# zhoubin-me/agent0

Hardware: AMD Instinct MI355X
Metric: env-frames/sec (learner FPS: transitions collected and saved to replay per second with the learner running, pre-frameskip) (higher is better)
Workload: dtype f32

## Files before the change

agent0_amd/csrc/encoder_fused.hip:

```cpp
#include "a0_internal.h"
#include "net_tables.h"
#include "operands.h"
#include "store_policy.h"
#include "update_tail.h"

#include <cstdlib>
#include <type_traits>

typedef float a0_acc4 __attribute__((ext_vector_type(4)));

struct a0_fused_args {
    const uint8_t* frames; const int* slot; long long sample_stride; int chan_off;
    const float *wt1, *wt2, *wt3;
    const float *wx2, *wx3;
    const float *b1, *b2, *b3;
    float *act1, *act2, *act3;
    int B;
    int C, H, W, H1, W1, H2, W2, H3, W3;
    int off_act1, off_act2, off_end;
    int rp1, rp2;
};

A0_HD void a0_fused_set_wt(a0_fused_args& P, const float* wt, int C) {
    const a0_wt_layout T{C};
// ... 357 lines not shown
    const float* bias; uint16_t* planes; float* glb; int N;
    A0_D void emit_n4(int m, int n0, const a0_acc4& acc, const float*) const {
        const a0_f4 bv = *(const a0_f4*)(bias + n0);
        float v[4] = {acc[0] + bv.x, acc[1] + bv.y, acc[2] + bv.z, acc[3] + bv.w};
#pragma unroll
        for (int r = 0; r < 4; ++r) v[r] = (v[r] < 0.f) ? 0.f : v[r];
        if (glb) *(a0_f4*)(glb + (unsigned)(m * N + n0)) = a0_f4{v[0], v[1], v[2], v[3]};
        uint2 hi, mid, lo;
        a0_split4(v, hi, mid, lo);
        const int oh = m / OWC;
        uint16_t* d = planes + oh * RP + (m - oh * OWC) * P + n0;
        *(uint2*)d = hi; *(uint2*)(d + term) = mid; *(uint2*)(d + 2 * term) = lo;
    }
};
struct EpiFwdT {
    static constexpr bool PER_ELEM = false;
    static constexpr bool ROW4 = false;
    static constexpr bool TR = true;
    const float* bias; float* glb; int N;
    A0_D void emit_n4(int m, int n0, const a0_acc4& acc, const float*) const {
        const a0_f4 bv = *(const a0_f4*)(bias + n0);
        float v[4] = {acc[0] + bv.x, acc[1] + bv.y, acc[2] + bv.z, acc[3] + bv.w};
#pragma unroll
        for (int r = 0; r < 4; ++r) v[r] = (v[r] < 0.f) ? 0.f : v[r];
        *(a0_f4*)(glb + (unsigned)(m * N + n0)) = a0_f4{v[0], v[1], v[2], v[3]};
    }
};

template <int ORD, int N, int WN, int MBT, int R, int LR, class AFX, class EPI, class Between>
A0_D void a0_conv_stage_x9k(const AFX& af, int M, a0_wring9<N, WN, R, A0_FUSED_WAVES / WN>& ring, const EPI& epi, float* xch0, float* xch1, Between&& between) {
    constexpr int WK = A0_FUSED_WAVES / WN, HB0 = (MBT + 1) / 2, HB1 = MBT / 2;
    static_assert(WK == 2 && N == 16 * WN && HB1 >= 1 && EPI::TR && LR >= 1 && LR <= 16, "tile shape");
    const int tid = threadIdx.x, lane = tid & 63;
    const int wave = __builtin_amdgcn_readfirstlane(tid >> 6);
    const int wn = wave % WN, wk = wave / WN;
    const int q = lane >> 4, r16 = lane & 15;
    const int MB = (M + 15) >> 4, NSTW = ring.nst;
    int rows[MBT];
#pragma unroll
    for (int i = 0; i < MBT; ++i) {
        const int m = i * 16 + r16;
        rows[i] = af.row(m < M ? m : 0) + 8 * q;
    }
    a0_acc4 acc[MBT];
#pragma unroll
    for (int i = 0; i < MBT; ++i) acc[i] = a0_acc4{0.f, 0.f, 0.f, 0.f};
    uint4 a[2][HB0][3];
    auto fetch = [&](int slot, int h, int off) {
#pragma unroll
        for (int i = 0; i < HB0; ++i)
            if (h * HB0 + i < MBT) {
#pragma unroll
                for (int t = 0; t < 3; ++t) a[slot][i][t] = *(const uint4*)(af.planes + rows[h * HB0 + i] + off + t * AFX::term);
            }
    };
    fetch(0, 0, af.step_off(wk));
    __builtin_amdgcn_s_waitcnt(0x0F70);
#pragma unroll 1
    for (int tb = 0; tb < NSTW; tb += R) {
#pragma unroll
        for (int u = 0; u < R; ++u) {
            const int st = wk + WK * (tb + u);
            const int off = af.step_off(st), offn = af.step_off(tb + u + 1 < NSTW ? st + WK : st);
#pragma unroll
            for (int h = 0; h < 2; ++h) {
                if (h == 0) fetch(1, 1, off);
                else fetch(0, 0, offn);
                __builtin_amdgcn_sched_barrier(0);
#pragma unroll
                for (int ta = 0; ta < 3; ++ta)
#pragma unroll
                    for (int tw = 0; tw < 3; ++tw)
#pragma unroll
                        for (int i = 0; i < HB0; ++i) {
                            if (ta + tw > ORD || h * HB0 + i >= MBT) continue;
                            const a0_u32x4 av = {a[h][i][ta].x, a[h][i][ta].y, a[h][i][ta].z, a[h][i][ta].w};
                            const a0_u32x4 bv = {ring.v[u][0][tw].x, ring.v[u][0][tw].y, ring.v[u][0][tw].z, ring.v[u][0][tw].w};
                            acc[h * HB0 + i] = __builtin_amdgcn_mfma_f32_16x16x32_bf16(__builtin_bit_cast(a0_bf16x8, bv), __builtin_bit_cast(a0_bf16x8, av), acc[h * HB0 + i], 0, 0, 0);
                        }
                __builtin_amdgcn_sched_barrier(0);
            }
            ring.fill(u);
            __builtin_amdgcn_sched_barrier(0);
        }
    }
    between();
    a0_acc4* x0 = (a0_acc4*)xch0;
    a0_acc4* x1 = (a0_acc4*)xch1;
    constexpr int P1 = (HB1 - 1) * 64 + 4 * LR;
    const int last = q * LR + r16;
    const int n0 = wn * 16 + 4 * q;
    float pe[EPI::PER_ELEM ? HB0 : 1][4];
    auto send = [&](auto mine) {
        constexpr int H = decltype(mine)::value;
        if constexpr (EPI::PER_ELEM) {
#pragma unroll
            for (int i = 0; i < (H == 0 ? HB0 : HB1); ++i) {
                const int m = (H * HB0 + i) * 16 + r16;
                const a0_f4 v = epi.pre_elem4(m < M ? m : M - 1, n0);
                pe[i][0] = v.x; pe[i][1] = v.y; pe[i][2] = v.z; pe[i][3] = v.w;
            }
        }
        if constexpr (H == 1) {
#pragma unroll
            for (int i = 0; i < HB0; ++i) x0[(wn * HB0 + i) * 64 + lane] = acc[i];
        } else {
#pragma unroll
            for (int i = 0; i < HB1; ++i) {
                if (i < HB1 - 1) x1[wn * P1 + i * 64 + lane] = acc[HB0 + i];
                else if (r16 < LR) x1[wn * P1 + (HB1 - 1) * 64 + last] = acc[HB0 + i];
            }
        }
    };
    auto recv = [&](auto mine) {
        constexpr int H = decltype(mine)::value;
#pragma unroll
        for (int i = 0; i < (H == 0 ? HB0 : HB1); ++i) {
            const int mb = H * HB0 + i;
            const int m = mb * 16 + r16;
            if constexpr (H == 0) acc[mb] += x0[(wn * HB0 + i) * 64 + lane];
            else {
                if (i < HB1 - 1) acc[mb] += x1[wn * P1 + i * 64 + lane];
                else if (r16 < LR) acc[mb] += x1[wn * P1 + (HB1 - 1) * 64 + last];
            }
            if (mb < MB && m < M) epi.emit_n4(m, n0, acc[mb], EPI::PER_ELEM ? pe[EPI::PER_ELEM ? i : 0] : nullptr);
        }
    };
    if (wk == 0) send(std::integral_constant<int, 0>{});
    else send(std::integral_constant<int, 1>{});
    __syncthreads();
    if (wk == 0) recv(std::integral_constant<int, 0>{});
    else recv(std::integral_constant<int, 1>{});
    __syncthreads();
}
constexpr int A0_P1X = 40, A0_P2X = 80;
constexpr int A0_RP1X = 20 * A0_P1X + 8;
constexpr int A0_RP2X = 9 * A0_P2X + 96;

constexpr int A0_R1 = 4, A0_R2 = 4, A0_R3 = 6;

template <int MBW1, int MBW2, int MBW3, int WC, bool X9, bool LOOP = false, int ORD = 4>
__global__ __launch_bounds__(A0_FUSED_THREADS) void a0_encoder_fused_kernel(a0_fused_args P);

constexpr int A0_X9_BIAS_OFF = 2 * 4 * 84 * 84 + 3 * 20 * A0_RP1X * 2;
constexpr int A0_RK2 = 2, A0_RK3 = 3;
constexpr int A0_X9_XCH0 = 3 * 9 * A0_RP2X * 2;
constexpr int A0_X9_XCH1 = A0_X9_BIAS_OFF + 160 * 4;
static_assert(A0_X9_XCH0 + 4 * 3 * 1024 <= 2 * 4 * 84 * 84, "conv2 exchange region 0 fits into the image");
constexpr int A0_X9_LDS_BYTES = A0_X9_XCH1 + 4 * (2 * 64 + 4) * 16;
static_assert(A0_X9_LDS_BYTES <= 160 * 1024, "LDS");
static_assert(A0_FUSED_WAVES == 8, "N-stationary stages: four waves along N, two along K");
typedef a0_wring9<64, 4, A0_RK2, 2> a0_ring2_t;
typedef a0_wring9<64, 4, A0_RK3, 2> a0_ring3_t;
template <int ORD, bool LOOP>
A0_D void a0_x9_conv23(const a0_fused_args& P, int b, unsigned char* smem, float* bias_lds, a0_wring1<A0_R1>& ring1, a0_ring2_t& ring2, a0_ring3_t& ring3) {
    const int obs_bytes = P.C * P.H * P.W;
    const int M2 = P.H2 * P.W2, M3 = P.H3 * P.W3;
    uint16_t* a1p = (uint16_t*)(smem + 2 * obs_bytes);
    constexpr int term1 = 20 * A0_RP1X, term2 = 9 * A0_RP2X;
    uint16_t* a2p = (uint16_t*)smem;
    typedef EpiFwdX<9, A0_P2X, A0_RP2X, term2> E2X;
    const AF2X<term1> f2{a1p, A0_RP1X, P.W2, A0_P1X};
    const E2X e2{bias_lds + 32, a2p, P.act2 ? P.act2 + (long long)b * M2 * 64 : nullptr, 64};
    const AF3X<term2> f3{a2p, A0_RP2X, P.W3, A0_P2X};
    const EpiFwdT e3{bias_lds + 96, P.act3 + (long long)b * M3 * 64, 64};
    a0_conv_stage_x9k<ORD, 64, 4, 6, A0_RK2, 1>(f2, M2, ring2, e2, (float*)(smem + A0_X9_XCH0), (float*)(smem + A0_X9_XCH1), [&] { ring3.prologue(); });
    a0_conv_stage_x9k<ORD, 64, 4, 4, A0_RK3, 16>(f3, M3, ring3, e3, (float*)a1p, (float*)a1p + 4 * 2 * 256, [&] { if (LOOP) ring1.prologue(); });
}

A0_D void a0_bytes16_to_img(uint16_t* img, int idx16, const uint4& v) {
    const uint32_t w[4] = {v.x, v.y, v.z, v.w};
    uint32_t o[8];
#pragma unroll
    for (int k = 0; k < 4; ++k) {
        const uint32_t f0 = __float_as_uint((float)(w[k] & 0xffu)), f1 = __float_as_uint((float)((w[k] >> 8) & 0xffu));
        const uint32_t f2 = __float_as_uint((float)((w[k] >> 16) & 0xffu)), f3 = __float_as_uint((float)(w[k] >> 24));
        o[2 * k] = __builtin_amdgcn_perm(f1, f0, 0x07060302u);
        o[2 * k + 1] = __builtin_amdgcn_perm(f3, f2, 0x07060302u);
    }
    ((uint4*)img)[2 * idx16] = uint4{o[0], o[1], o[2], o[3]};
    ((uint4*)img)[2 * idx16 + 1] = uint4{o[4], o[5], o[6], o[7]};
}

template <int ORD, bool LOOP>
A0_D void a0_encoder_fused_x9_body(const a0_fused_args& P, int bid, int nblk) {
    extern __shared__ __attribute__((aligned(16))) unsigned char smem[];
    uint16_t* img = (uint16_t*)smem;
    const int obs_bytes = P.C * P.H * P.W;
    const int M1 = P.H1 * P.W1;
    uint16_t* a1p = (uint16_t*)(smem + 2 * obs_bytes);
    constexpr int term1 = 20 * A0_RP1X;
    typedef EpiFwdX<20, A0_P1X, A0_RP1X, term1> E1X;
    a0_wring1<A0_R1> ring1;
    a0_ring2_t ring2;
    a0_ring3_t ring3;
    ring1.init(P.wt1, P.C);
    ring2.init(P.wx2, 512);
    ring3.init(P.wx3, 576);
    ring1.prologue();
    constexpr int MBW1X = (25 + A0_WMG1 - 1) / A0_WMG1;
    a0_pre<32, 2, MBW1X, E1X> pre1;
    float* bias_lds = (float*)(smem + A0_X9_BIAS_OFF);
    if (threadIdx.x < 160) bias_lds[threadIdx.x] = threadIdx.x < 32 ? P.b1[threadIdx.x] : threadIdx.x < 96 ? P.b2[threadIdx.x - 32] : P.b3[threadIdx.x - 96];
    for (int b = bid; b < P.B; b += nblk) {
        const long long s = P.slot ? (long long)P.slot[b] : (long long)b;
        const uint4* src = (const uint4*)(P.frames + s * P.sample_stride + P.chan_off);
        constexpr int TRIPS = 4;
        const int n16 = obs_bytes >> 4;
        for (int i0 = threadIdx.x; i0 < n16; i0 += TRIPS * A0_FUSED_THREADS) {
            uint4 v[TRIPS];
#pragma unroll
            for (int j = 0; j < TRIPS; ++j) {
                const int i = i0 + j * A0_FUSED_THREADS;
                v[j] = src[i < n16 ? i : n16 - 1];
            }
#pragma unroll
            for (int j = 0; j < TRIPS; ++j) {
                const int i = i0 + j * A0_FUSED_THREADS;
                a0_bytes16_to_img(img, i < n16 ? i : n16 - 1, v[j]);
            }
        }
        __syncthreads();
        const E1X e1{bias_lds, a1p, P.act1 ? P.act1 + (long long)b * M1 * 32 : nullptr, 32};
        const int wmg1 = __builtin_amdgcn_readfirstlane(threadIdx.x >> 6) / 2;
        if (MBW1X > 1 && wmg1 + (MBW1X - 1) * A0_WMG1 >= ((M1 + 15) >> 4))
            a0_conv1_stage<(MBW1X > 1 ? MBW1X - 1 : 1), A0_R1, 84>(img, P.H * P.W, P.W, P.W1, M1, ring1, e1, pre1, [&] { ring2.prologue(); });
        else
            a0_conv1_stage<MBW1X, A0_R1, 84>(img, P.H * P.W, P.W, P.W1, M1, ring1, e1, pre1, [&] { ring2.prologue(); });
        a0_x9_conv23<ORD, LOOP>(P, b, smem, bias_lds, ring1, ring2, ring3);
        if constexpr (!LOOP) break;
    }
}

#include "actor_tail.h"
typedef a0_st_nt a0_step_row_store;
struct a0_step_enc_args { const float *wt, *b1, *b2, *b3; float* act3; };
template <int ORD>
__global__ __launch_bounds__(A0_FUSED_THREADS) void a0_actor_dist_step_enc_kernel(a0_dtenv_args Q, a0_step_enc_args N) {
    __shared__ int s_chase_cell;
    extern __shared__ __attribute__((aligned(16))) unsigned char smem[];
    unsigned long long v_wt = (unsigned long long)N.wt, v_b1 = (unsigned long long)N.b1, v_b2 = (unsigned long long)N.b2, v_b3 = (unsigned long long)N.b3,
                       v_a3 = (unsigned long long)N.act3, v_obs = (unsigned long long)Q.obs_out;
    A0_TO_VGPR(v_wt); A0_TO_VGPR(v_b1); A0_TO_VGPR(v_b2); A0_TO_VGPR(v_b3); A0_TO_VGPR(v_a3); A0_TO_VGPR(v_obs);
    int v_E = Q.E;
    A0_TO_VGPR(v_E);
    a0_actor_dist_tail_env_body(Q, (float*)smem, &s_chase_cell);
    __syncthreads();
    auto uni = [](unsigned long long v) {
        return ((unsigned long long)(unsigned)__builtin_amdgcn_readfirstlane((int)(v >> 32)) << 32) | (unsigned long long)(unsigned)__builtin_amdgcn_readfirstlane((int)(v & 0xffffffffull));
    };
    const float* wt = (const float*)uni(v_wt);
    a0_fused_args P;
    P.frames = (const uint8_t*)uni(v_obs); P.slot = nullptr; P.sample_stride = 4 * 84 * 84; P.chan_off = 0;
    a0_fused_set_wt(P, wt, 4);
    P.b1 = (const float*)uni(v_b1); P.b2 = (const float*)uni(v_b2); P.b3 = (const float*)uni(v_b3);
    P.act1 = nullptr; P.act2 = nullptr; P.act3 = (float*)uni(v_a3); P.B = __builtin_amdgcn_readfirstlane(v_E);
    P.C = 4; P.H = 84; P.W = 84; P.H1 = 20; P.W1 = 20; P.H2 = 9; P.W2 = 9; P.H3 = 7; P.W3 = 7;
    P.off_act1 = 0; P.off_act2 = 0; P.off_end = 0; P.rp1 = 0; P.rp2 = 0;
    a0_encoder_fused_x9_body<ORD, false>(P, (int)blockIdx.x, (int)gridDim.x);
}

template <int MBW, class EPI, class Mid, class Between>
A0_D void a0_conv1_stage_split(const uint16_t* img, a0_wring1<A0_R1>& ring, const EPI& epi, bool first_before_mid, Mid&& mid, Between&& between) {
    static_assert(A0_R1 == 4 && EPI::TR, "ring of four steps, transposed accumulators");
    constexpr int HW = 84 * 84, W = 84, W1 = 20, M = 400, MB = 25;
    const int tid = threadIdx.x, lane = tid & 63;
    const int wave = __builtin_amdgcn_readfirstlane(tid >> 6);
    const int wn = wave % 2, wmg = wave / 2;
    const int q = lane >> 4, r16 = lane & 15;
    int rows[MBW];
#pragma unroll
    for (int i = 0; i < MBW; ++i) {
        int m = (wmg + i * A0_WMG1) * 16 + r16;
        m = m < M ? m : 0;
        const int oh = m / W1, ow = m - oh * W1;
        rows[i] = (4 * oh + q) * W + 4 * ow;
    }
    a0_acc4 acc[MBW];
#pragma unroll
    for (int i = 0; i < MBW; ++i) acc[i] = a0_acc4{0.f, 0.f, 0.f, 0.f};
    uint2 a[2][MBW][2];
    auto fetch = [&](int slot, int off) {
#pragma unroll
        for (int i = 0; i < MBW; ++i) {
            a[slot][i][0] = *(const uint2*)(img + rows[i] + off);
            a[slot][i][1] = *(const uint2*)(img + rows[i] + off + 4);
        }
    };
    auto off_of = [&](int st) { return (st >> 1) * HW + (st & 1) * 4 * W; };
    auto step = [&](auto UC, int off_next) {
        constexpr int u = decltype(UC)::value;
        fetch((u + 1) & 1, off_next);
        __builtin_amdgcn_sched_barrier(0);
#pragma unroll
        for (int s3 = 0; s3 < 3; ++s3)
#pragma unroll
            for (int i = 0; i < MBW; ++i) {
                const a0_u32x4 av = {a[u & 1][i][0].x, a[u & 1][i][0].y, a[u & 1][i][1].x, a[u & 1][i][1].y};
                const a0_u32x4 bv = {ring.v[u][s3].x, ring.v[u][s3].y, ring.v[u][s3].z, ring.v[u][s3].w};
                acc[i] = __builtin_amdgcn_mfma_f32_16x16x32_bf16(__builtin_bit_cast(a0_bf16x8, bv), __builtin_bit_cast(a0_bf16x8, av), acc[i], 0, 0, 0);
            }
        __builtin_amdgcn_sched_barrier(0);
        ring.fill(u);
        __builtin_amdgcn_sched_barrier(0);
    };
    typedef std::integral_constant<int, 0> U0; typedef std::integral_constant<int, 1> U1; typedef std::integral_constant<int, 2> U2; typedef std::integral_constant<int, 3> U3;
    auto steps05 = [&] {
        fetch(0, off_of(0));
        __builtin_amdgcn_s_waitcnt(0x0F70);
        step(U0{}, off_of(1)); step(U1{}, off_of(2)); step(U2{}, off_of(3)); step(U3{}, off_of(4));
        step(U0{}, off_of(5)); step(U1{}, off_of(5));
    };
    if (first_before_mid) steps05();
    mid();
    if (!first_before_mid) steps05();
    fetch(0, off_of(6));
    __builtin_amdgcn_s_waitcnt(0x0F70);
    step(U2{}, off_of(7)); step(U3{}, off_of(7));
    between();
#pragma unroll
    for (int i = 0; i < MBW; ++i) {
        const int mb = wmg + i * A0_WMG1;
        if (mb < MB) {
            const int m = mb * 16 + r16;
            if (m < M) epi.emit_n4(m, wn * 16 + 4 * q, acc[i], nullptr);
        }
    }
    __syncthreads();
}

struct TailScalar {
    typedef a0_qenv_args Args;
    static A0_D void run(const a0_qenv_args& Q, uint32_t e, uint32_t g, long long steps, unsigned long long off_a, unsigned long long off_u, float eps, long long slot, const a0_u4& x,
                         bool chase, int lane, float* w2s , float* raw, int* s_chase_cell_p) {
        const int NQ = Q.A + (Q.dueling ? 1 : 0);
// ... 46 lines not shown
    if (tid < 160) bias_lds[tid] = tid < 32 ? P.b1[tid] : tid < 96 ? P.b2[tid - 32] : P.b3[tid - 96];
    unsigned long long v_wx2 = (unsigned long long)P.wx2, v_wx3 = (unsigned long long)P.wx3;
    A0_TO_VGPR(v_wx2); A0_TO_VGPR(v_wx3);
    uint32_t g = Q.g; long long steps = Q.steps, start = Q.start; unsigned long long off_a = Q.off_a, off_u = Q.off_u; float eps = Q.eps;
    if (Q.ctrl) {
        g += (uint32_t)Q.ctrl[A0_CTRL_ENV_STEP]; steps += Q.ctrl[A0_CTRL_ACTOR_STEPS]; start += Q.ctrl[A0_CTRL_REPLAY_SLOT];
        off_a += (unsigned long long)Q.ctrl[A0_CTRL_RNG_ACTION]; off_u += (unsigned long long)Q.ctrl[A0_CTRL_RNG_UNIFORM];
    }
    eps = a0_env_eps(eps, Q.eps_ptr, e);
    const long long slot = (start + e) % Q.cap;
    uint32_t e_v = e;
    asm volatile("" : "+v"(e_v));
    const a0_u4 x = a0_philox4x32_10(e_v, g, 0u, 0x454E56u, (uint32_t)Q.env_seed, (uint32_t)(Q.env_seed >> 32) ^ Q.rank);
    const bool term = __builtin_amdgcn_readfirstlane((int)((x.y % 500u) == 0u)) != 0;
    const bool chase = Q.task == A0_ENV_TASK_CHASE;
    const bool early = !(chase && term);
    const int j = tid - 64;
    auto has_group = [&] { int jj = j; asm volatile("" : "+v"(jj)); return wave != 0 && jj < G16; };
    const uint32_t pbase = (uint32_t)Q.env_seed ^ a0_env_mix32(e * 0x9E3779B1u + g);
    uint4* out16 = (uint4*)(Q.obs_out + (size_t)e * 4 * HW) + j;
    uint4* row16 = (uint4*)(Q.frames + slot * (8LL * HW)) + j;
    A0_TO_VGPR(out16); A0_TO_VGPR(row16);
    float* act3_v = N.act3;
    A0_TO_VGPR(act3_v);
    auto new_group = [&](uint32_t by, uint32_t bx) {
        uint32_t w[4];
#pragma unroll
        for (int k = 0; k < 4; ++k) {
            const uint32_t p = 16u * (uint32_t)j + 4u * (uint32_t)k;
            w[k] = (uint32_t)a0_env_pixel(pbase, by, bx, p, chase) | ((uint32_t)a0_env_pixel(pbase, by, bx, p + 1, chase) << 8) |
                   ((uint32_t)a0_env_pixel(pbase, by, bx, p + 2, chase) << 16) | ((uint32_t)a0_env_pixel(pbase, by, bx, p + 3, chase) << 24);
        }
        return uint4{w[0], w[1], w[2], w[3]};
    };
    auto put = [&](int c, const uint4 v) {
        out16[c * G16] = v; a0_store16<a0_step_row_store>(row16 + (4 + c) * G16, v);
        a0_bytes16_to_img(img, c * G16 + j, v);
    };
    __shared__ int s_staged;
    if (tid == 0) s_staged = 0;
    __syncthreads();
    uint4 keep[9];
    if (wave == 0) {
        TAIL::run(Q, e, g, steps, off_a, off_u, eps, slot, x, chase, lane, (float*)a1p, raw, &s_chase_cell);
    } else {
        if (has_group()) {
            const uint4* in16 = (const uint4*)(Q.obs_in + (size_t)e * 4 * HW) + j;
            A0_TO_VGPR(in16);
            const uint4 i0 = in16[0], i1 = in16[G16], i2 = in16[2 * G16], i3 = in16[3 * G16];
            if (Q.obs0 == Q.obs_in) { keep[0] = i0; keep[1] = i1; keep[2] = i2; keep[3] = i3; }
            else {
                const uint4* o016 = (const uint4*)(Q.obs0 + (size_t)e * 4 * HW) + j;
                A0_TO_VGPR(o016);
                keep[0] = o016[0]; keep[1] = o016[G16]; keep[2] = o016[2 * G16]; keep[3] = o016[3 * G16];
            }
            if (!chase) {
                const uint4 nw = new_group((3u * g + 11u * e) % 77u, (5u * g + 7u * e) % 77u);
                if (term) { keep[4] = nw; keep[5] = nw; keep[6] = nw; } else { keep[4] = i1; keep[5] = i2; keep[6] = i3; }
                keep[7] = nw;
                for (int c = 0; c < 4; ++c) a0_bytes16_to_img(img, c * G16 + j, keep[4 + c]);
            } else if (!term) {
                keep[4] = i1; keep[5] = i2; keep[6] = i3;
                for (int c = 0; c < 3; ++c) a0_bytes16_to_img(img, c * G16 + j, keep[4 + c]);
            }
        }
        asm volatile("s_waitcnt lgkmcnt(0)" ::: "memory");
        if (lane == 0) atomicAdd(&s_staged, 1);
        while (__builtin_amdgcn_readfirstlane(*(volatile int*)&s_staged) < A0_FUSED_WAVES - 1) __builtin_amdgcn_s_sleep(1);
    }
    auto early_stores = [&] {
        if (has_group()) {
#pragma unroll
            for (int c = 0; c < 4; ++c) a0_store16<a0_step_row_store>(row16 + c * G16, keep[c]);
            const int nc = !chase ? 4 : (!term ? 3 : 0);
#pragma unroll
            for (int c = 0; c < 4; ++c)
                if (c < nc) { out16[c * G16] = keep[4 + c]; a0_store16<a0_step_row_store>(row16 + (4 + c) * G16, keep[4 + c]); }
        }
    };
    auto mid = [&] {
        if (wave != 0) early_stores();
        __syncthreads();
        if (chase) {
            if (has_group()) {
                uint32_t by, bx;
                a0_chase_pos(s_chase_cell, by, bx);
                const uint4 nw = new_group(by, bx);
                if (term) { put(0, nw); put(1, nw); put(2, nw); }
                put(3, nw);
            }
            __syncthreads();
        }
    };
    auto uni = [](unsigned long long v) {
        return ((unsigned long long)(unsigned)__builtin_amdgcn_readfirstlane((int)(v >> 32)) << 32) | (unsigned long long)(unsigned)__builtin_amdgcn_readfirstlane((int)(v & 0xffffffffull));
    };
    ring2.init((const float*)uni(v_wx2), 512);
    ring3.init((const float*)uni(v_wx3), 576);
    typedef EpiFwdX<20, A0_P1X, A0_RP1X, 20 * A0_RP1X> E1X;
    const E1X e1{bias_lds, a1p, nullptr, 32};
    constexpr int MBW1X = (25 + A0_WMG1 - 1) / A0_WMG1;
    const bool before = early && wave != 0;
    if (MBW1X > 1 && wave / 2 + (MBW1X - 1) * A0_WMG1 >= 25)
        a0_conv1_stage_split<(MBW1X > 1 ? MBW1X - 1 : 1)>(img, ring1, e1, before, mid, [&] { ring2.prologue(); });
    else
        a0_conv1_stage_split<MBW1X>(img, ring1, e1, before, mid, [&] { ring2.prologue(); });
    P.act3 = (float*)uni((unsigned long long)act3_v);
    a0_x9_conv23<ORD, false>(P, (int)e, smem, bias_lds, ring1, ring2, ring3);
}

template <int ORD>
__global__ __launch_bounds__(A0_FUSED_THREADS) void a0_actor_step_enc2_kernel(a0_qenv_args Q, a0_step_enc_args N) { a0_actor_step_enc2_body<ORD, TailScalar>(Q, N); }

static bool a0_fused_layout(int C, int H, int W, a0_fused_args& P, size_t& lds_bytes);
int a0_actor_dist_step_enc_launch(const a0_dtenv_args& Q, size_t tail_lds, const float* wt, const a0_encoder_weights* w, float* act3, hipStream_t st) {
    a0_fused_args P;
    size_t lds = 0;
    if (!wt || !w || !w->b1 || !w->b2 || !w->b3 || !act3 || !a0_fused_layout(4, 84, 84, P, lds)) return a0_fail(A0_EINVAL, "a0_actor_dist_tail_env_step_enc: bad encoder argument");
    if (P.H1 != 20 || P.W1 != 20 || P.H2 != 9 || P.W2 != 9 || P.H3 != 7 || P.W3 != 7) return a0_fail(A0_EINVAL, "a0_actor_dist_tail_env_step_enc: geometry");
    const a0_step_enc_args N{wt, w->b1, w->b2, w->b3, act3};
    lds = A0_X9_LDS_BYTES > tail_lds ? (size_t)A0_X9_LDS_BYTES : tail_lds;
    if (lds > 160 * 1024 - 64) return a0_fail(A0_EINVAL, "a0_actor_dist_tail_env_step_enc: head too wide for LDS");
    const int six = a0_x9_products_now() == 6;
    auto kern = six ? a0_actor_dist_step_enc_kernel<2> : a0_actor_dist_step_enc_kernel<4>;
    static size_t configured[2] = {0, 0};
    if (lds > configured[six]) {
        if (hipFuncSetAttribute((const void*)kern, hipFuncAttributeMaxDynamicSharedMemorySize, (int)lds) != hipSuccess)
            return a0_fail(A0_EINVAL, "a0_actor_dist_tail_env_step_enc: LDS");
        configured[six] = lds;
    }
    A0_LAUNCH_PROBED(A0_TAG_ACTOR_STEP_ENC, 2.0 * (400.0 * 32 * 256 + 81.0 * 64 * 512 + 49.0 * 64 * 576) * Q.E, kern, dim3(Q.E), dim3(A0_FUSED_THREADS), lds, st, Q, N);
    return a0_fail_hip((int)hipGetLastError(), "a0_actor_dist_tail_env_step_enc");
}
int a0_actor_step_enc_launch(const a0_qenv_args& Q, const float* wt, const a0_encoder_weights* w, float* act3, hipStream_t st) {
    a0_fused_args P;
    size_t lds = 0;
    if (!wt || !w || !w->b1 || !w->b2 || !w->b3 || !act3 || !a0_fused_layout(4, 84, 84, P, lds)) return a0_fail(A0_EINVAL, "a0_actor_qhead_env_step_enc: bad encoder argument");
    if (P.H1 != 20 || P.W1 != 20 || P.H2 != 9 || P.W2 != 9 || P.H3 != 7 || P.W3 != 7) return a0_fail(A0_EINVAL, "a0_actor_qhead_env_step_enc: geometry");
    const a0_step_enc_args N{wt, w->b1, w->b2, w->b3, act3};
    const size_t tail_lds = (size_t)(Q.A + (Q.dueling ? 1 : 0)) * 512 * sizeof(float);
    lds = A0_X9_LDS_BYTES > tail_lds ? (size_t)A0_X9_LDS_BYTES : tail_lds;
    const int six = a0_x9_products_now() == 6;
    auto kern = six ? a0_actor_step_enc2_kernel<2> : a0_actor_step_enc2_kernel<4>;
    static size_t configured[2] = {0, 0};
    if (lds > configured[six]) {
        if (hipFuncSetAttribute((const void*)kern, hipFuncAttributeMaxDynamicSharedMemorySize, (int)lds) != hipSuccess)
            return a0_fail(A0_EINVAL, "a0_actor_qhead_env_step_enc: LDS");
        configured[six] = lds;
    }
    A0_LAUNCH_PROBED(A0_TAG_ACTOR_STEP_ENC, 2.0 * (400.0 * 32 * 256 + 81.0 * 64 * 512 + 49.0 * 64 * 576) * Q.E, kern, dim3(Q.E), dim3(A0_FUSED_THREADS), lds, st, Q, N);
    return a0_fail_hip((int)hipGetLastError(), "a0_actor_qhead_env_step_enc");
}

struct a0_fused_multi_args { a0_fused_args p[3]; int first[4]; };
template <int ORD>
__global__ __launch_bounds__(A0_FUSED_THREADS) void a0_encoder_fused_multi_kernel(a0_fused_multi_args M) {
    const int bid = (int)blockIdx.x;
    const int k = bid >= M.first[2] ? 2 : (bid >= M.first[1] ? 1 : 0);
    a0_encoder_fused_x9_body<ORD, true>(M.p[k], bid - M.first[k], M.first[k + 1] - M.first[k]);
}

template <int MBW1, int MBW2, int MBW3, int WC, bool X9, bool LOOP, int ORD>
__global__ __launch_bounds__(A0_FUSED_THREADS) void a0_encoder_fused_kernel(a0_fused_args P) {
    if constexpr (X9) {
        static_assert(MBW1 == 7 && MBW2 == 3 && MBW3 == 2 && WC == 84, "the split-operand body is written for the 4 x 84 x 84 geometry");
        a0_encoder_fused_x9_body<ORD, LOOP>(P, (int)blockIdx.x, (int)gridDim.x);
        return;
    }
    extern __shared__ __attribute__((aligned(16))) unsigned char smem[];
    uint16_t* img = (uint16_t*)smem;
    float* fl = (float*)smem;
    float* act1 = fl + P.off_act1;
    float* act2 = fl + P.off_act2;
    const int obs_bytes = P.C * P.H * P.W;
    const int M1 = P.H1 * P.W1, M2 = P.H2 * P.W2, M3 = P.H3 * P.W3;
    a0_wring1<A0_R1> ring1;
    a0_wring<64, 4, A0_R2> ring2;
    a0_wring<64, 4, A0_R3> ring3;
    ring1.init(P.wt1, P.C);
    ring2.init(P.wt2, 512);
    ring3.init(P.wt3, 576);
    ring1.prologue();
    constexpr int OW1 = WC == 84 ? 20 : 0, OW2 = WC == 84 ? 9 : 0;
    a0_pre<32, 2, MBW1, EpiFwd<OW1>> pre1;
    a0_pre<64, 4, MBW2, EpiFwd<OW2>> pre2;
    a0_pre<64, 4, MBW3, EpiFwd<0>> pre3;
    pre1.load(EpiFwd<OW1>{P.b1, nullptr, 0, 0, 1, nullptr, 32}, M1);
    pre2.load(EpiFwd<OW2>{P.b2, nullptr, 0, 0, 1, nullptr, 64}, M2);
    pre3.load(EpiFwd<0>{P.b3, nullptr, 0, 0, 1, nullptr, 64}, M3);
    for (int b = blockIdx.x; b < P.B; b += gridDim.x) {
        const long long s = P.slot ? (long long)P.slot[b] : (long long)b;
        const uint4* src = (const uint4*)(P.frames + s * P.sample_stride + P.chan_off);
        constexpr int TRIPS = 4;
        const int n16 = obs_bytes >> 4;
        for (int i0 = threadIdx.x; i0 < n16; i0 += TRIPS * A0_FUSED_THREADS) {
            uint4 v[TRIPS];
#pragma unroll
            for (int j = 0; j < TRIPS; ++j) {
                const int i = i0 + j * A0_FUSED_THREADS;
                v[j] = src[i < n16 ? i : n16 - 1];
            }
#pragma unroll
            for (int j = 0; j < TRIPS; ++j) {
                const int i = i0 + j * A0_FUSED_THREADS;
                a0_bytes16_to_img(img, i < n16 ? i : n16 - 1, v[j]);
            }
        }
        __syncthreads();
        const EpiFwd<OW1> e1{P.b1, act1, A0_P1, P.rp1, P.W1, P.act1 ? P.act1 + (long long)b * M1 * 32 : nullptr, 32};
        const int wmg1 = __builtin_amdgcn_readfirstlane(threadIdx.x >> 6) / 2;
        if (MBW1 > 1 && wmg1 + (MBW1 - 1) * 4 >= ((M1 + 15) >> 4))
            a0_conv1_stage<(MBW1 > 1 ? MBW1 - 1 : 1), A0_R1, WC>(img, P.H * P.W, P.W, P.W1, M1, ring1, e1, pre1, [&] { ring2.prologue(); });
        else
            a0_conv1_stage<MBW1, A0_R1, WC>(img, P.H * P.W, P.W, P.W1, M1, ring1, e1, pre1, [&] { ring2.prologue(); });
        AF2 f2{act1, P.rp1, P.W2};
        const EpiFwd<OW2> e2{P.b2, act2, A0_P2, P.rp2, P.W2, P.act2 ? P.act2 + (long long)b * M2 * 64 : nullptr, 64};
        a0_conv_stage<64, 4, MBW2, 3, A0_R2>(f2, M2, 512, ring2, e2, pre2, [&] { ring3.prologue(); });
        AF3 f3{act2, P.rp2, P.W3};
        const EpiFwd<0> e3{P.b3, nullptr, 0, 0, 1, P.act3 + (long long)b * M3 * 64, 64};
        a0_conv_stage<64, 4, MBW3, 3, A0_R3>(f3, M3, 576, ring3, e3, pre3, [&] { ring1.prologue(); });
    }
}

struct a0_dgrad_args {
    const float *d3, *act1, *act2;
    float *d2, *d1;
    const float *wd3, *wd2;
    int B;
};
constexpr int A0_RPDA = 11 * A0_P2X + 96, A0_RPDB = 11 * A0_P2X + 48;
constexpr int A0_DTERMA = 11 * A0_RPDA, A0_DTERMB = 11 * A0_RPDB;
struct AFD3X {
    static constexpr int term = A0_DTERMA;
    const uint16_t* planes;
    A0_D int row(int m) const { const int oh = m / 9, ow = m - oh * 9; return oh * A0_RPDA + ow * A0_P2X; }
    A0_D int step_off(int st) const { const int tap = st >> 1; return (tap / 3) * A0_RPDA + (tap % 3) * A0_P2X + 32 * (st & 1); }
};
struct AFD2X {
    static constexpr int term = A0_DTERMB;
    const uint16_t* planes;
    A0_D int row(int m) const { const int oh = m / 10, ow = m - oh * 10; return oh * A0_RPDB + ow * A0_P2X; }
    A0_D int step_off(int st) const { const int cell = st >> 1; return (cell >> 1) * A0_RPDB + (cell & 1) * A0_P2X + 32 * (st & 1); }
};
struct EpiBwd3X {
    static constexpr bool PER_ELEM = true;
    static constexpr bool ROW4 = false;
    static constexpr bool TR = true;
    const float* mask; float* dst; uint16_t* planes;
    A0_D a0_f4 pre_elem4(int m, int n0) const { return *(const a0_f4*)(mask + (unsigned)(m * 64 + n0)); }
    A0_D void emit_n4(int m, int n0, const a0_acc4& acc, const float* pre) const {
        float v[4];
#pragma unroll
        for (int r = 0; r < 4; ++r) v[r] = pre[r] > 0.f ? acc[r] : 0.f;
        *(a0_f4*)(dst + (unsigned)(m * 64 + n0)) = a0_f4{v[0], v[1], v[2], v[3]};
        uint2 hi, mid, lo;
        a0_split4(v, hi, mid, lo);
        const int oh = m / 9, ow = m - oh * 9;
        uint16_t* d = planes + (oh + 1) * A0_RPDB + (ow + 1) * A0_P2X + n0;
        *(uint2*)d = hi; *(uint2*)(d + A0_DTERMB) = mid; *(uint2*)(d + 2 * A0_DTERMB) = lo;
    }
};
static_assert((A0_RPDB % 4) == 0 && (A0_DTERMB % 4) == 0 && (A0_P2X % 4) == 0, "8-byte aligned plane writes");
struct EpiBwdPair {
    static constexpr bool PER_ELEM = true;
    static constexpr bool ROW4 = false;
    static constexpr bool TR = true;
    const float* mask; float* dst; int p0;
    A0_D unsigned gi(int m, int n0) const {
        const int p = p0 + (n0 >> 5), oh = m / 10, ow = m - oh * 10;
        return (unsigned)(((oh * 2 + (p >> 1)) * 20 + ow * 2 + (p & 1)) * 32 + (n0 & 31));
    }
    A0_D a0_f4 pre_elem4(int m, int n0) const { return *(const a0_f4*)(mask + gi(m, n0)); }
    A0_D void emit_n4(int m, int n0, const a0_acc4& acc, const float* pre) const {
        *(a0_f4*)(dst + gi(m, n0)) = a0_f4{pre[0] > 0.f ? acc[0] : 0.f, pre[1] > 0.f ? acc[1] : 0.f, pre[2] > 0.f ? acc[2] : 0.f, pre[3] > 0.f ? acc[3] : 0.f};
    }
};
template <int ORD>
__global__ __launch_bounds__(A0_FUSED_THREADS) void a0_encoder_dgrad_fused_x9_kernel(a0_dgrad_args P) {
    extern __shared__ __attribute__((aligned(16))) unsigned char smem[];
    uint16_t* plA = (uint16_t*)smem;
    uint16_t* plB = plA + 3 * A0_DTERMA;
    for (int i = threadIdx.x; i < 3 * (A0_DTERMA + A0_DTERMB) / 2; i += A0_FUSED_THREADS) ((uint32_t*)smem)[i] = 0u;
    float* const xch0 = (float*)(smem + 3 * (A0_DTERMA + A0_DTERMB) * 2);
    float* const xch1 = xch0 + 4 * 4 * 256;
    const int lane = threadIdx.x & 63, wave = __builtin_amdgcn_readfirstlane(threadIdx.x >> 6), wn = wave & 3, wk = wave >> 2;
    a0_wring9<64, 4, 3, 2> ring3;
    a0_wring9<64, 4, 2, 2> ringq[2];
    ring3.init(P.wd3, 576);
    ring3.prologue();
    const uint4* const wq = (const uint4*)P.wd2 + (((wn & 1) * 16 + (lane & 15)) * 4 + (lane >> 4)) * 3 + (wn >> 1) * 3072 + wk * 384;
    __syncthreads();
    for (int b = blockIdx.x; b < P.B; b += gridDim.x) {
        const a0_f4* src = (const a0_f4*)(P.d3 + (long long)b * 49 * 64);
        for (int i = threadIdx.x; i < 49 * 16; i += A0_FUSED_THREADS) {
            const a0_f4 v = src[i];
            const int pos = i >> 4, c4 = (i & 15) * 4, h = pos / 7, w = pos - h * 7;
            const float x[4] = {v.x, v.y, v.z, v.w};
            uint2 hi, mid, lo;
            a0_split4(x, hi, mid, lo);
            uint16_t* d = plA + (h + 2) * A0_RPDA + (w + 2) * A0_P2X + c4;
            *(uint2*)(d) = hi; *(uint2*)(d + A0_DTERMA) = mid; *(uint2*)(d + 2 * A0_DTERMA) = lo;
        }
        __syncthreads();
        const AFD3X f3{plA};
        const AFD2X f2{plB};
        const EpiBwd3X e3{P.act2 + (long long)b * 81 * 64, P.d2 + (long long)b * 81 * 64, plB};
        const EpiBwdPair e2a{P.act1 + (long long)b * 400 * 32, P.d1 + (long long)b * 400 * 32, 0};
        const EpiBwdPair e2b{P.act1 + (long long)b * 400 * 32, P.d1 + (long long)b * 400 * 32, 2};
        a0_conv_stage_x9k<ORD, 64, 4, 6, 3, 1>(f3, 81, ring3, e3, xch0, xch1, [&] { ringq[0].init_at(wq, 4, 768); ringq[0].prologue(); });
        a0_conv_stage_x9k<ORD, 64, 4, 7, 2, 4>(f2, 100, ringq[0], e2a, xch0, xch1, [&] { ringq[1].init_at(wq + 2 * 3072, 4, 768); ringq[1].prologue(); });
        a0_conv_stage_x9k<ORD, 64, 4, 7, 2, 4>(f2, 100, ringq[1], e2b, xch0, xch1, [&] { ring3.prologue(); });
    }
}

__global__ void a0_conv_wt_kernel(const float* __restrict__ w1, const float* __restrict__ w2, const float* __restrict__ w3, float* __restrict__ wt, int K1,
                                  float* __restrict__ wt2, const int* __restrict__ state, int* __restrict__ commit) {
    const bool mirror = wt2 != nullptr && state[4] != 0;
    if (commit != nullptr && blockIdx.x == 0 && threadIdx.x == 0) { commit[1] = commit[5]; commit[0] = 0; }
    const a0_wt_layout T{K1 / 64};
    const int i = blockIdx.x * blockDim.x + threadIdx.x;
    if (i >= T.total()) return;
    uint32_t out = 0;
    if (i >= T.conv2() && i < T.conv2x()) {
        const bool c3 = i >= T.conv3();
        const int e = i - (c3 ? T.conv3() : T.conv2());
        const int j = e & 3, q = (e >> 2) & 3, n = (e >> 4) & 63, k = 16 * (e >> 10) + 4 * j + q;
        out = __float_as_uint(c3 ? w3[n * 576 + k] : w2[n * 512 + k]);
    } else {
        enum { CONV1, CONV2, CONV3, DGRAD3, DGRAD2 } seg;
        int e, N = 64, phase = 0;
        if (i < T.conv2()) { seg = CONV1; e = i; N = 32; }
        else if (i < T.conv3x()) { seg = CONV2; e = i - T.conv2x(); }
        else if (i < T.dgrad3x()) { seg = CONV3; e = i - T.conv3x(); }
        else if (i < T.dgrad2x()) { seg = DGRAD3; e = i - T.dgrad3x(); }
        else { seg = DGRAD2; e = i - T.dgrad2x(); phase = e / T.n_dgrad2x_phase; e -= phase * T.n_dgrad2x_phase; N = 32; }
        const int pair = e & 3, f = e >> 2, s = f % 3, q = (f / 3) & 3, n = (f / 12) % N, t = f / (12 * N);
        for (int h = 0; h < 2; ++h) {
            const int k = 32 * t + 8 * q + 2 * pair + h, cell = k >> 6, co = k & 63;
            float w;
            if (seg == CONV1) w = w1[n * K1 + k] / 255.0f;
            else if (seg == CONV2) w = w2[n * 512 + k];
            else if (seg == CONV3) w = w3[n * 576 + k];
            else if (seg == DGRAD3) {
                const int kh = 2 - cell / 3, kw = 2 - cell % 3;
                w = w3[co * 576 + (kh * 3 + kw) * 64 + n];
            } else {
                const int kh = (phase >> 1) + 2 * (1 - (cell >> 1)), kw = (phase & 1) + 2 * (1 - (cell & 1));
                w = w2[co * 512 + (kh * 4 + kw) * 32 + n];
            }
            out |= a0_bf16_term(w, s) << (16 * h);
        }
    }
    *(uint32_t*)(wt + i) = out;
    if (mirror) *(uint32_t*)(wt2 + i) = out;
}

extern "C" long long a0_net_conv_wt_floats(int C) { return a0_wt_layout{C}.total(); }

extern "C" int a0_net_conv_wt_refresh(const a0_encoder_weights* w, int C, float* wt, void* stream) {
    if (!w || !w->w1 || !w->w2 || !w->w3 || !wt || C < 1) return a0_fail(A0_EINVAL, "a0_net_conv_wt_refresh: bad argument");
    const long long n = a0_net_conv_wt_floats(C);
    hipLaunchKernelGGL(a0_conv_wt_kernel, dim3((unsigned)((n + 255) / 256)), dim3(256), 0, (hipStream_t)stream, w->w1, w->w2, w->w3, wt, C * 64, (float*)nullptr,
                       (const int*)nullptr, (int*)nullptr);
    return a0_fail_hip((int)hipGetLastError(), "a0_net_conv_wt_refresh");
}

extern "C" int a0_net_conv_wt_refresh_sync(const a0_encoder_weights* w, int C, float* wt, float* wt_target, const int* state, void* stream) {
    if (!w || !w->w1 || !w->w2 || !w->w3 || !wt || !wt_target || !state || C < 1) return a0_fail(A0_EINVAL, "a0_net_conv_wt_refresh_sync: bad argument");
    const long long n = a0_net_conv_wt_floats(C);
    hipLaunchKernelGGL(a0_conv_wt_kernel, dim3((unsigned)((n + 255) / 256)), dim3(256), 0, (hipStream_t)stream, w->w1, w->w2, w->w3, wt, C * 64, wt_target, state, (int*)nullptr);
    return a0_fail_hip((int)hipGetLastError(), "a0_net_conv_wt_refresh_sync");
}

int a0_conv_wt_refresh_commit(const a0_encoder_weights* w, int C, float* wt, float* wt_target, int* state, hipStream_t st) {
    if (!w || !w->w1 || !w->w2 || !w->w3) return a0_fail(A0_EINVAL, "a0_adam_step_sync_wt: encoder weights missing");
    const long long n = a0_net_conv_wt_floats(C);
    hipLaunchKernelGGL(a0_conv_wt_kernel, dim3((unsigned)((n + 255) / 256)), dim3(256), 0, st, w->w1, w->w2, w->w3, wt, C * 64, wt_target, (const int*)state, state);
    return a0_fail_hip((int)hipGetLastError(), "a0_adam_step_sync_wt");
}

static bool a0_fused_layout(int C, int H, int W, a0_fused_args& P, size_t& lds_bytes) {
    a0_net_core n;
    if (!a0_net_core_init(n, C, H, W)) return false;
    const int M1 = n.H1 * n.W1, M2 = n.H2 * n.W2, M3 = n.H3 * n.W3;
    if (M1 > 7 * 4 * 16 || M2 > 4 * 2 * 16 || M3 > 2 * 2 * 16) return false;
    if ((C * 2) % A0_R1 || (W & 3)) return false;
    const int obs_bytes = C * H * W;
    if (obs_bytes % 16) return false;
    P.C = C; P.H = H; P.W = W; P.H1 = n.H1; P.W1 = n.W1; P.H2 = n.H2; P.W2 = n.W2; P.H3 = n.H3; P.W3 = n.W3;
    P.rp1 = n.W1 * A0_P1;
    while ((P.rp1 - n.W2) & 15) ++P.rp1;
    P.rp2 = n.W2 * A0_P2;
    while ((P.rp2 - 2 * n.W3) & 31) ++P.rp2;
    P.off_act1 = obs_bytes / 2;
    P.off_act2 = P.off_act1 + ((n.H1 * P.rp1 + 3) & ~3);
    P.off_end = P.off_act2 + ((n.H2 * P.rp2 + 3) & ~3);
    lds_bytes = (size_t)P.off_end * 4;
    return lds_bytes <= 160 * 1024;
}

static bool a0_fused_fill(int C, int H, int W, const float* wt, const a0_encoder_weights* w, const a0_frames_arg* f, float* act1, float* act2, float* act3, int B,
                          a0_fused_args& P, size_t& lds_bytes) {
    if (!a0_fused_layout(C, H, W, P, lds_bytes)) return false;
    P.frames = f->frames; P.slot = f->slot; P.sample_stride = f->sample_stride; P.chan_off = f->chan_off;
    a0_fused_set_wt(P, wt, C);
    P.b1 = w->b1; P.b2 = w->b2; P.b3 = w->b3;
    P.act1 = act1; P.act2 = act2; P.act3 = act3; P.B = B;
    return true;
}

extern "C" int a0_net_encoder_fused_supported(int C, int H, int W) {
    a0_fused_args P; size_t lds;
    return a0_fused_layout(C, H, W, P, lds) ? 1 : 0;
}

extern "C" int a0_net_encoder_fwd_fused(int C, int H, int W, const float* wt, const a0_encoder_weights* w, const a0_frames_arg* f, int B,
                                        float* act1, float* act2, float* act3, void* stream) {
    A0_TRY
    if (!wt || !w || !w->b1 || !w->b2 || !w->b3 || !f || !f->frames || !act3 || B < 1) return a0_fail(A0_EINVAL, "a0_net_encoder_fwd_fused: bad argument");
    a0_fused_args P;
    size_t lds = 0;
    if (!a0_fused_fill(C, H, W, wt, w, f, act1, act2, act3, B, P, lds)) return a0_fail(A0_EINVAL, "a0_net_encoder_fwd_fused: observation shape not supported by the fused kernel");
    if ((f->sample_stride % 16) || (f->chan_off % 16) || (((uintptr_t)f->frames) % 16)) return a0_fail(A0_EINVAL, "a0_net_encoder_fwd_fused: frames must be 16-byte aligned");
    const int mb1 = (P.H1 * P.W1 + 15) / 16, mb2 = (P.H2 * P.W2 + 15) / 16, mb3 = (P.H3 * P.W3 + 15) / 16;
    const bool standard = ((mb1 + 3) / 4 == 7) && ((mb2 + 1) / 2 == 3) && ((mb3 + 1) / 2 == 2) && W == 84;
    const bool x9 = standard && H == 84 && C == 4;
    int which = x9 ? 2 : (standard ? 1 : 0);
    if (x9) lds = A0_X9_LDS_BYTES;
    static_assert(3 * 9 * A0_RP2X * 2 <= 2 * 4 * 84 * 84, "the act2 term planes fit into the dead image");
    const int gridx = (which == 2 && B > 256) ? 256 : B;
    if (which == 2 && gridx < B) which = 3;
    static size_t configured[6] = {0, 0, 0, 0, 0, 0};
    const int six = a0_x9_products_now() == 6;
    if (six && which >= 2) which += 2;
    typedef void (*a0_enc_kern)(a0_fused_args);
    const a0_enc_kern fn = which == 5 ? a0_encoder_fused_kernel<7, 3, 2, 84, true, true, 2> : which == 4 ? a0_encoder_fused_kernel<7, 3, 2, 84, true, false, 2>
                         : which == 3 ? a0_encoder_fused_kernel<7, 3, 2, 84, true, true> : which == 2 ? a0_encoder_fused_kernel<7, 3, 2, 84, true>
                         : which == 1 ? a0_encoder_fused_kernel<7, 3, 2, 84, false> : a0_encoder_fused_kernel<7, 4, 2, 0, false>;
    if (lds > configured[which]) {
        A0_HIP_THROW(hipFuncSetAttribute((const void*)fn, hipFuncAttributeMaxDynamicSharedMemorySize, (int)lds));
        configured[which] = lds;
    }
    const double per_obs = 2.0 * ((double)P.H1 * P.W1 * 32 * (P.C * 64) + (double)P.H2 * P.W2 * 64 * 512 + (double)P.H3 * P.W3 * 64 * 576);
    A0_LAUNCH_PROBED(A0_TAG_ENCODER_FUSED, per_obs * B, fn, dim3((which == 3 || which == 5) ? gridx : B), dim3(A0_FUSED_THREADS), lds, (hipStream_t)stream, P);
    A0_HIP_THROW(hipGetLastError());
    return A0_OK;
    A0_CATCH
}

extern "C" int a0_net_encoder_fwd_fused_multi(int C, int H, int W, int n, const a0_encoder_pass* pass, void* stream) {
    A0_TRY
    if (n < 1 || n > 3 || !pass) return a0_fail(A0_EINVAL, "a0_net_encoder_fwd_fused_multi: 1 to 3 passes");
    if (!(C == 4 && H == 84 && W == 84)) return a0_fail(A0_EINVAL, "a0_net_encoder_fwd_fused_multi: 4 x 84 x 84 observations on the split-operand kernel only");
    a0_fused_multi_args M;
    size_t lds = 0;
    long long total = 0;
    for (int i = 0; i < n; ++i) {
        const a0_encoder_pass& q = pass[i];
        if (!q.wt || !q.w || !q.w->b1 || !q.w->b2 || !q.w->b3 || !q.f || !q.f->frames || !q.act3 || q.B < 1) return a0_fail(A0_EINVAL, "a0_net_encoder_fwd_fused_multi: bad pass");
        if ((q.f->sample_stride % 16) || (q.f->chan_off % 16) || (((uintptr_t)q.f->frames) % 16)) return a0_fail(A0_EINVAL, "a0_net_encoder_fwd_fused_multi: frames must be 16-byte aligned");
        if (!a0_fused_fill(C, H, W, q.wt, q.w, q.f, q.act1, q.act2, q.act3, q.B, M.p[i], lds))
            return a0_fail(A0_EINVAL, "a0_net_encoder_fwd_fused_multi: observation shape");
        total += q.B;
    }
    for (int i = n; i < 3; ++i) M.p[i] = M.p[0];
    int grid = (int)(total < 256 ? total : 256), used = 0;
    if (grid < n) grid = n;
    for (int i = 0; i < n; ++i) {
        M.first[i] = used;
        int share = (i == n - 1) ? grid - used : (int)((long long)grid * pass[i].B / total);
        if (share < 1) share = 1;
        if (share > pass[i].B) share = pass[i].B;
        used += share;
    }
    for (int i = n; i <= 3; ++i) M.first[i] = 0x7fffffff;
    M.first[n] = used;
    lds = A0_X9_LDS_BYTES;
    const int six = a0_x9_products_now() == 6;
    auto kern = six ? a0_encoder_fused_multi_kernel<2> : a0_encoder_fused_multi_kernel<4>;
    static bool configured[2] = {false, false};
    if (!configured[six]) {
        A0_HIP_THROW(hipFuncSetAttribute((const void*)kern, hipFuncAttributeMaxDynamicSharedMemorySize, (int)lds));
        configured[six] = true;
    }
    const a0_fused_args& P0 = M.p[0];
    const double per_obs = 2.0 * ((double)P0.H1 * P0.W1 * 32 * (P0.C * 64) + (double)P0.H2 * P0.W2 * 64 * 512 + (double)P0.H3 * P0.W3 * 64 * 576);
    A0_LAUNCH_PROBED(A0_TAG_ENCODER_FUSED, per_obs * (double)total, kern, dim3(used), dim3(A0_FUSED_THREADS), lds, (hipStream_t)stream, M);
    A0_HIP_THROW(hipGetLastError());
    return A0_OK;
    A0_CATCH
}

extern "C" int a0_net_encoder_dgrad_fused_supported(int C, int H, int W) { return (C >= 1 && H == 84 && W == 84) ? 1 : 0; }

extern "C" int a0_net_encoder_dgrad_fused(int C, int H, int W, const float* wt, const float* d3, const float* act1, const float* act2, int B, float* d2,
                                          float* d1, void* stream) {
    A0_TRY
    if (!wt || !d3 || !act1 || !act2 || !d2 || !d1 || B < 1) return a0_fail(A0_EINVAL, "a0_net_encoder_dgrad_fused: bad argument");
    if (!a0_net_encoder_dgrad_fused_supported(C, H, W)) return a0_fail(A0_EINVAL, "a0_net_encoder_dgrad_fused: 84x84 observations only");
    a0_dgrad_args P;
    P.d3 = d3; P.act1 = act1; P.act2 = act2; P.d2 = d2; P.d1 = d1; P.B = B;
    P.wd3 = wt + a0_wt_layout{C}.dgrad3x(); P.wd2 = wt + a0_wt_layout{C}.dgrad2x();
    const size_t lds = (size_t)3 * (A0_DTERMA + A0_DTERMB) * 2 + (4 * 4 + 4 * 3) * 1024;
    static bool configured[2] = {false, false};
    const int six = a0_x9_products_now() == 6;
    auto fn = six ? a0_encoder_dgrad_fused_x9_kernel<2> : a0_encoder_dgrad_fused_x9_kernel<4>;
    if (!configured[six]) {
        A0_HIP_THROW(hipFuncSetAttribute((const void*)fn, hipFuncAttributeMaxDynamicSharedMemorySize, (int)lds));
        configured[six] = true;
    }
    const int gridx = B > 256 ? 256 : B;
    A0_LAUNCH_PROBED(A0_TAG_ENCODER_DGRAD_FUSED, 2.0 * (81.0 * 64 * 576 + 400.0 * 32 * 256) * B, fn, dim3(gridx), dim3(A0_FUSED_THREADS), lds, (hipStream_t)stream, P);
    A0_HIP_THROW(hipGetLastError());
    return A0_OK;
    A0_CATCH
}
```

Baseline: 2.519 million.

## Stride blocks across concatenated passes in multi-pass fused encoder kernel

Replaces the static per-pass block partition of the multi-pass encoder kernel with a grid-stride loop over the concatenated observations of all passes. Each block walks observations with stride equal to the grid size and crosses pass boundaries by reloading weight rings and biases only when the pass changes. The aim is to balance load when pass sizes are uneven and to remove the rounding of per-pass block shares. The cost is more complex control flow, with bias and ring reinitialisation happening inside the loop.

```diff
diff --git a/agent0_amd/csrc/encoder_fused.hip b/agent0_amd/csrc/encoder_fused.hip
--- a/agent0_amd/csrc/encoder_fused.hip
+++ b/agent0_amd/csrc/encoder_fused.hip
@@ -533,8 +533,8 @@
 static_assert(A0_FUSED_WAVES == 8, "N-stationary stages: four waves along N, two along K");
 typedef a0_wring9<64, 4, A0_RK2, 2> a0_ring2_t;
 typedef a0_wring9<64, 4, A0_RK3, 2> a0_ring3_t;
-template <int ORD, bool LOOP>
-A0_D void a0_x9_conv23(const a0_fused_args& P, int b, unsigned char* smem, float* bias_lds, a0_wring1<A0_R1>& ring1, a0_ring2_t& ring2, a0_ring3_t& ring3) {
+template <int ORD, class Between3>
+A0_D void a0_x9_conv23_then(const a0_fused_args& P, int b, unsigned char* smem, float* bias_lds, a0_ring2_t& ring2, a0_ring3_t& ring3, Between3&& between3) {
     const int obs_bytes = P.C * P.H * P.W;
     const int M2 = P.H2 * P.W2, M3 = P.H3 * P.W3;
     uint16_t* a1p = (uint16_t*)(smem + 2 * obs_bytes);
@@ -546,7 +546,11 @@
     const AF3X<term2> f3{a2p, A0_RP2X, P.W3, A0_P2X};
     const EpiFwdT e3{bias_lds + 96, P.act3 + (long long)b * M3 * 64, 64};
     a0_conv_stage_x9k<ORD, 64, 4, 6, A0_RK2, 1>(f2, M2, ring2, e2, (float*)(smem + A0_X9_XCH0), (float*)(smem + A0_X9_XCH1), [&] { ring3.prologue(); });
-    a0_conv_stage_x9k<ORD, 64, 4, 4, A0_RK3, 16>(f3, M3, ring3, e3, (float*)a1p, (float*)a1p + 4 * 2 * 256, [&] { if (LOOP) ring1.prologue(); });
+    a0_conv_stage_x9k<ORD, 64, 4, 4, A0_RK3, 16>(f3, M3, ring3, e3, (float*)a1p, (float*)a1p + 4 * 2 * 256, between3);
+}
+template <int ORD, bool LOOP>
+A0_D void a0_x9_conv23(const a0_fused_args& P, int b, unsigned char* smem, float* bias_lds, a0_wring1<A0_R1>& ring1, a0_ring2_t& ring2, a0_ring3_t& ring3) {
+    a0_x9_conv23_then<ORD>(P, b, smem, bias_lds, ring2, ring3, [&] { if (LOOP) ring1.prologue(); });
 }
 
 A0_D void a0_bytes16_to_img(uint16_t* img, int idx16, const uint4& v) {
@@ -562,6 +566,45 @@
     ((uint4*)img)[2 * idx16] = uint4{o[0], o[1], o[2], o[3]};
     ((uint4*)img)[2 * idx16 + 1] = uint4{o[4], o[5], o[6], o[7]};
 }
+
+template <int ORD, class Gathered, class Between3>
+A0_D void a0_x9_observation(const a0_fused_args& P, int b, unsigned char* smem, int obs_bytes, int M1, float* bias_lds, a0_wring1<A0_R1>& ring1, a0_ring2_t& ring2, a0_ring3_t& ring3,
+                            Gathered&& gathered, Between3&& between3) {
+    uint16_t* img = (uint16_t*)smem;
+    uint16_t* a1p = (uint16_t*)(smem + 2 * obs_bytes);
+    constexpr int term1 = 20 * A0_RP1X;
+    typedef EpiFwdX<20, A0_P1X, A0_RP1X, term1> E1X;
+    constexpr int MBW1X = (25 + A0_WMG1 - 1) / A0_WMG1;
+    a0_pre<32, 2, MBW1X, E1X> pre1;
+    const long long s = P.slot ? (long long)P.slot[b] : (long long)b;
+    const uint4* src = (const uint4*)(P.frames + s * P.sample_stride + P.chan_off);
+    constexpr int TRIPS = 4;
+    const int n16 = obs_bytes >> 4;
+    for (int i0 = threadIdx.x; i0 < n16; i0 += TRIPS * A0_FUSED_THREADS) {
+        uint4 v[TRIPS];
+#pragma unroll
+        for (int j = 0; j < TRIPS; ++j) {
+            const int i = i0 + j * A0_FUSED_THREADS;
+            v[j] = src[i < n16 ? i : n16 - 1];
+        }
+#pragma unroll
+        for (int j = 0; j < TRIPS; ++j) {
+            const int i = i0 + j * A0_FUSED_THREADS;
+            a0_bytes16_to_img(img, i < n16 ? i : n16 - 1, v[j]);
+        }
+    }
+    gathered();
+    __syncthreads();
+    const E1X e1{bias_lds, a1p, P.act1 ? P.act1 + (long long)b * M1 * 32 : nullptr, 32};
+    const int wmg1 = __builtin_amdgcn_readfirstlane(threadIdx.x >> 6) / 2;
+    if (MBW1X > 1 && wmg1 + (MBW1X - 1) * A0_WMG1 >= ((M1 + 15) >> 4))
+        a0_conv1_stage<(MBW1X > 1 ? MBW1X - 1 : 1), A0_R1, 84>(img, P.H * P.W, P.W, P.W1, M1, ring1, e1, pre1, [&] { ring2.prologue(); });
+    else
+        a0_conv1_stage<MBW1X, A0_R1, 84>(img, P.H * P.W, P.W, P.W1, M1, ring1, e1, pre1, [&] { ring2.prologue(); });
+    a0_x9_conv23_then<ORD>(P, b, smem, bias_lds, ring2, ring3, between3);
+}
+
+A0_D float a0_x9_bias_at(const a0_fused_args& P, int i) { return i < 32 ? P.b1[i] : i < 96 ? P.b2[i - 32] : P.b3[i - 96]; }
 
 template <int ORD, bool LOOP>
 A0_D void a0_encoder_fused_x9_body(const a0_fused_args& P, int bid, int nblk) {
@@ -914,12 +957,50 @@
     return a0_fail_hip((int)hipGetLastError(), "a0_actor_qhead_env_step_enc");
 }
 
-struct a0_fused_multi_args { a0_fused_args p[3]; int first[4]; };
+struct a0_fused_multi_args { a0_fused_args p[3]; int n; };
 template <int ORD>
 __global__ __launch_bounds__(A0_FUSED_THREADS) void a0_encoder_fused_multi_kernel(a0_fused_multi_args M) {
-    const int bid = (int)blockIdx.x;
-    const int k = bid >= M.first[2] ? 2 : (bid >= M.first[1] ? 1 : 0);
-    a0_encoder_fused_x9_body<ORD, true>(M.p[k], bid - M.first[k], M.first[k + 1] - M.first[k]);
+    extern __shared__ __attribute__((aligned(16))) unsigned char smem[];
+    const int grid = (int)gridDim.x, tid = (int)threadIdx.x;
+    const int B0 = M.p[0].B, B1 = M.n > 1 ? M.p[1].B : 0, B2 = M.n > 2 ? M.p[2].B : 0;
+    auto size_of = [&](int k) { return k == 0 ? B0 : k == 1 ? B1 : B2; };
+    int g = (int)blockIdx.x, k = 0, G = 0;
+    while (g >= G + size_of(k)) { G += size_of(k); ++k; }
+    a0_wring1<A0_R1> ring1;
+    a0_ring2_t ring2;
+    a0_ring3_t ring3;
+    ring1.init(M.p[k].wt1, 4);
+    ring1.prologue();
+    float* bias_lds = (float*)(smem + A0_X9_BIAS_OFF);
+    float bias = tid < 160 ? a0_x9_bias_at(M.p[k], tid) : 0.f;
+    a0_fused_args P;
+    P.C = 4; P.H = 84; P.W = 84; P.H1 = 20; P.W1 = 20; P.H2 = 9; P.W2 = 9; P.H3 = 7; P.W3 = 7;
+    P.off_act1 = 0; P.off_act2 = 0; P.off_end = 0; P.rp1 = 0; P.rp2 = 0;
+    bool entered = true;
+#pragma unroll 1
+    for (;;) {
+        if (entered) {
+            const a0_fused_args& Q = M.p[k];
+            P.frames = Q.frames; P.slot = Q.slot; P.sample_stride = Q.sample_stride; P.chan_off = Q.chan_off;
+            P.act1 = Q.act1; P.act2 = Q.act2; P.act3 = Q.act3; P.B = Q.B;
+            ring2.init(Q.wx2, 512);
+            ring3.init(Q.wx3, 576);
+        }
+        const int gn = g + grid;
+        int kn = k, Gn = G;
+        if (gn >= G + P.B) do { Gn += size_of(kn); ++kn; } while (kn < M.n && gn >= Gn + size_of(kn));
+        a0_x9_observation<ORD>(P, g - G, smem, 4 * 84 * 84, 400, bias_lds, ring1, ring2, ring3, [&] { if (entered && tid < 160) bias_lds[tid] = bias; }, [&] {
+            if (kn == k) ring1.prologue();
+            else if (kn < M.n) {
+                ring1.init(M.p[kn].wt1, 4);
+                ring1.prologue();
+                if (tid < 160) bias = a0_x9_bias_at(M.p[kn], tid);
+            }
+        });
+        if (kn >= M.n) break;
+        entered = kn != k;
+        g = gn; k = kn; G = Gn;
+    }
 }
 
 template <int MBW1, int MBW2, int MBW3, int WC, bool X9, bool LOOP, int ORD>
@@ -1225,18 +1306,10 @@
             return a0_fail(A0_EINVAL, "a0_net_encoder_fwd_fused_multi: observation shape");
         total += q.B;
     }
+    if (total > 0x7fffffff - 256) return a0_fail(A0_EINVAL, "a0_net_encoder_fwd_fused_multi: too many observations");
     for (int i = n; i < 3; ++i) M.p[i] = M.p[0];
-    int grid = (int)(total < 256 ? total : 256), used = 0;
-    if (grid < n) grid = n;
-    for (int i = 0; i < n; ++i) {
-        M.first[i] = used;
-        int share = (i == n - 1) ? grid - used : (int)((long long)grid * pass[i].B / total);
-        if (share < 1) share = 1;
-        if (share > pass[i].B) share = pass[i].B;
-        used += share;
-    }
-    for (int i = n; i <= 3; ++i) M.first[i] = 0x7fffffff;
-    M.first[n] = used;
+    M.n = n;
+    const int grid = (int)(total < 256 ? total : 256);
     lds = A0_X9_LDS_BYTES;
     const int six = a0_x9_products_now() == 6;
     auto kern = six ? a0_encoder_fused_multi_kernel<2> : a0_encoder_fused_multi_kernel<4>;
@@ -1247,7 +1320,7 @@
     }
     const a0_fused_args& P0 = M.p[0];
     const double per_obs = 2.0 * ((double)P0.H1 * P0.W1 * 32 * (P0.C * 64) + (double)P0.H2 * P0.W2 * 64 * 512 + (double)P0.H3 * P0.W3 * 64 * 576);
-    A0_LAUNCH_PROBED(A0_TAG_ENCODER_FUSED, per_obs * (double)total, kern, dim3(used), dim3(A0_FUSED_THREADS), lds, (hipStream_t)stream, M);
+    A0_LAUNCH_PROBED(A0_TAG_ENCODER_FUSED, per_obs * (double)total, kern, dim3(grid), dim3(A0_FUSED_THREADS), lds, (hipStream_t)stream, M);
     A0_HIP_THROW(hipGetLastError());
     return A0_OK;
     A0_CATCH
```

Result: no change. 2.528 million (median of 4 runs) (+0.3%).
